# numz/ComfyUI-SeedVR2_VideoUpscaler

Hardware: AMD Instinct MI355X
Metric: upscaled frames/sec (720p->4K, SeedVR2-3B) (higher is better)
Workload: dtype bf16; 1 GPU; cfg3: SeedVR2-3B 32-frame 720p->4K clip (padded to 33 = 4n+1 for encode + DiT, 32 decoded), VAE tiled 1024/128; vae_tiled=True, parallelism=dp1, weights=random-init SeedVR2-3B + video_vae_v3 architecture (seeded)

## Files before the change

comfyui-seedvr2_videoupscaler_amd/csrc/svr_conv_halo2.hip:

```cpp
#include "svr_common.h"
#include "../../include/seedvr2_hip.h"
#include <type_traits>

namespace svr {

constexpr int CG_TX = 32, CG_HX = CG_TX + 2;
constexpr int CG_BUNIT = 128 * 64;
constexpr int CG_NB = 8;
constexpr int CG_D = 4;
static_assert(CG_D < CG_NB, "ring slot of unit k + D must not hold a unit still being read");

template <int TY, int MODE> struct cg_geom {
    static constexpr int MTW = MODE == 3 ? 8 : 4;
    static constexpr int NT = MODE == 3 ? 256 : TY * 32;
    static constexpr int HY = TY + 2;
    static constexpr int ROWS = CG_HX * HY;
    static constexpr int ACHUNKS = ROWS * 4;
    static constexpr int PIECES = (ACHUNKS + NT - 1) / NT;
    static constexpr int ABUF = MODE == 3 ? PIECES * NT * 16 : ROWS * 64;
    static constexpr int BOFF = 2 * ABUF;
    static constexpr int EP_ROWS = MODE ? 4 : 8;
    static constexpr int EP_BYTES = EP_ROWS * 32 * 528;
    static constexpr int THIN_PITCH = 272;
    static constexpr int MAIN = MODE == 2 ? TY * 32 * THIN_PITCH : (MODE == 1 || MODE == 3 ? BOFF : BOFF + CG_NB * CG_BUNIT);
    static constexpr int LDS = MAIN > EP_BYTES ? MAIN : EP_BYTES;
    static_assert(MODE == 3 || PIECES <= 7, "the next halo must have landed before interval 8");
};

template <int N> SVR_DEVICE void cg_wait_vmcnt() { asm volatile("s_waitcnt vmcnt(%0)" ::"n"(N) : "memory"); }
template <int OFF> SVR_DEVICE void cg_rd2(bf16x8 (&r)[2], unsigned a0) {
    const unsigned a1 = a0 ^ 32u;
    asm volatile("ds_read_b128 %0, %2 offset:%4\n\tds_read_b128 %1, %3 offset:%4"
                 : "=&v"(r[0]), "=&v"(r[1]) : "v"(a0), "v"(a1), "n"(OFF) : "memory");
}
template <int N> SVR_DEVICE void cg_wait_rows(bf16x8 (&a)[2]) {
    asm volatile("s_waitcnt lgkmcnt(%2)" : "+v"(a[0]), "+v"(a[1]) : "n"(N));
    __builtin_amdgcn_sched_barrier(0);
}
template <int N> SVR_DEVICE void cg_wait_rows(bf16x8 (&a)[2], bf16x8 (&b)[2]) {
    asm volatile("s_waitcnt lgkmcnt(%4)" : "+v"(a[0]), "+v"(a[1]), "+v"(b[0]), "+v"(b[1]) : "n"(N));
    __builtin_amdgcn_sched_barrier(0);
}
template <int N> SVR_DEVICE void cg_wait_rows(bf16x8 (&a)[2], bf16x8 (&b)[2], bf16x8 (&c)[2], bf16x8 (&d)[2], bf16x8 (&e)[2],
                                              bf16x8 (&f)[2], bf16x8 (&g)[2], bf16x8 (&h)[2]) {
    asm volatile("s_waitcnt lgkmcnt(%16)"
                 : "+v"(a[0]), "+v"(a[1]), "+v"(b[0]), "+v"(b[1]), "+v"(c[0]), "+v"(c[1]), "+v"(d[0]), "+v"(d[1]),
                   "+v"(e[0]), "+v"(e[1]), "+v"(f[0]), "+v"(f[1]), "+v"(g[0]), "+v"(g[1]), "+v"(h[0]), "+v"(h[1]) : "n"(N));
    __builtin_amdgcn_sched_barrier(0);
}
template <int N> SVR_DEVICE void cg_wait_w(bf16x8 (&w)[2][2]) {
    asm volatile("s_waitcnt vmcnt(%4)" : "+v"(w[0][0]), "+v"(w[0][1]), "+v"(w[1][0]), "+v"(w[1][1]) : "n"(N));
    __builtin_amdgcn_sched_barrier(0);
}

#ifdef SVR_ABLATIONS
__device__ unsigned long long g_conv_tl[4096][4];
__device__ unsigned long long g_conv_ep[4096][16];
#endif
template <int TY, int MODE, int DBG = 0>
__global__ __launch_bounds__((cg_geom<TY, MODE>::NT), (MODE == 3 ? 1 : 2)) void conv_halo2_kernel(const svr_gemm_args a, const int band_rows) {
#ifndef SVR_ABLATIONS
    static_assert(DBG == 0, "measurement variants (results invalid on purpose) exist only in -DSVR_ABLATIONS builds; the product library instantiates DBG = 0");
#endif
    typedef cg_geom<TY, MODE> G;
    constexpr bool WREG = MODE == 1 || MODE == 3, W8 = MODE == 3, THIN = MODE == 2;
    constexpr int CG_TY = TY, CG_ROWS = G::ROWS, CG_ABUF = G::ABUF, CG_ACHUNKS = G::ACHUNKS, CG_PIECES = G::PIECES,
                  CG_BOFF = G::BOFF, NT = G::NT;
    constexpr int MTW = G::MTW, NTW = 2;
    extern __shared__ __attribute__((aligned(16))) char smem[];
    typedef __attribute__((ext_vector_type(16))) float f32x16_t;

    const svr_conv_geom& g = a.conv;
    const int tid = threadIdx.x;
#ifdef SVR_ABLATIONS
    if constexpr ((DBG & 256) != 0) { if (tid == 0 && blockIdx.x < 4096) g_conv_tl[blockIdx.x][0] = __builtin_amdgcn_s_memtime(); }
#endif
    const int lane = tid & 63;
    const int wave = __builtin_amdgcn_readfirstlane(tid >> 6);
    const int grp = wave >> 2;
    const int wm = wave >> 1, wn = wave & 1;

    const int tiles_x = (g.W + CG_TX - 1) / CG_TX;
    const int tiles_y = (g.H + CG_TY - 1) / CG_TY;
    const int tiles_n = a.N / 128;
    int tl;
    {
        const int nwg = gridDim.x, bid = blockIdx.x;
        const int xcd = bid & 7, j = bid >> 3, q = nwg >> 3, r = nwg & 7;
        tl = (xcd < r ? xcd * (q + 1) : r * (q + 1) + (xcd - r) * q) + j;
    }
    const int tn = tl % tiles_n;
    int rr = tl / tiles_n;
    const int tx = rr % tiles_x; rr /= tiles_x;
    int ty, to;
    if (band_rows > 0 && band_rows < tiles_y) {
        const int per_band = band_rows * g.To;
        const int b = rr / per_band;
        const int rows_b = min(band_rows, tiles_y - b * band_rows);
        const int r2 = rr - b * per_band;
        to = r2 / rows_b;
        ty = b * band_rows + (r2 - to * rows_b);
    } else {
        ty = rr % tiles_y;
        to = rr / tiles_y;
    }
    const int y0 = ty * CG_TY, x0 = tx * CG_TX, n0 = tn * 128;

    const int cpk = THIN ? 1 : g.Cin / 32;
    const int nA = g.kt * cpk;
    const int P = nA * 9;
    const int64_t frame_bytes = (int64_t)g.H * g.W * g.Cin * 2;
    const int srow = tid >> 2, spos = tid & 3;
    const char* wbase = (const char*)a.W + (int64_t)(n0 + srow) * a.K * 2 + ((spos ^ ((srow >> 2) & 3)) * 16);
    uint32_t poff[CG_PIECES];
    uint32_t akeys = 0;
#pragma unroll
    for (int q = 0; q < CG_PIECES; ++q) {
        const int row = q * (NT / 4) + srow;
        const int hy = row / CG_HX, hx = row - hy * CG_HX;
        const int y = y0 - 1 + hy, x = x0 - 1 + hx;
        const bool ok = row < CG_ROWS && (unsigned)y < (unsigned)g.H && (unsigned)x < (unsigned)g.W;
        poff[q] = ok ? (uint32_t)(y * g.W + x) : 0xffffffffu;
        akeys |= (uint32_t)(spos ^ ((hx >> 2) & 3)) << (2 * q);
    }
    char* const wave_dst = smem + wave * 1024;

    auto frame_ptr = [&](int s) -> const char* {
        const int dt = s / cpk;
        const int c0 = (s - dt * cpk) * 32;
        int f = to + dt - g.pt;
        const char* basep = (const char*)a.A;
        if (f < 0) {
            if (g.halo != nullptr) { basep = (const char*)g.halo; f += g.halo_frames; }
            else f = 0;
        }
        return basep + (int64_t)f * frame_bytes + c0 * 2;
    };
    auto stage_a_piece = [&](auto qc, const char* fptr, int buf) {
        constexpr int Q = decltype(qc)::value;
        if (Q * NT + wave * 64 >= CG_ACHUNKS) return false;
        const int ck = (akeys >> (2 * Q)) & 3;
        const char* src = poff[Q] == 0xffffffffu ? (const char*)g.zeros
                                                 : fptr + ((int64_t)poff[Q] * g.Cin + ck * 8) * 2;
        if constexpr (!(DBG & 2))
            if (Q * NT + tid < CG_ACHUNKS) glds16(src, wave_dst + buf * CG_ABUF + Q * (NT * 16));
        return true;
    };
    auto stage_b = [&](int s, int tap, int slot) {
        const int dt = s / cpk;
        const int c0 = (s - dt * cpk) * 32;
        const int64_t koff = ((int64_t)(dt * 9 + tap) * g.Cin + c0) * 2;
        glds16(wbase + koff, wave_dst + CG_BOFF + slot * CG_BUNIT);
    };

    const int l31 = lane & 31, hi = lane >> 5;
    int rd_a0[3], rd_b0;
#pragma unroll
    for (int dx = 0; dx < 3; ++dx)
        rd_a0[dx] = (wm * MTW * CG_HX + l31) * 64 + ((hi ^ (((dx + l31) >> 2) & 3)) << 4);
    rd_b0 = CG_BOFF + (wn * 64 + l31) * 64 + ((hi ^ ((l31 >> 2) & 3)) << 4);

    f32x16_t acc[MTW][NTW];
#pragma unroll
    for (int y = 0; y < MTW; ++y)
#pragma unroll
        for (int z = 0; z < NTW; ++z)
#pragma unroll
            for (int e = 0; e < 16; ++e) acc[y][z][e] = 0.f;
    bf16x8 ar0[2], ar1[2], ar2[2], ar3[2], ar4[2], ar5[2], wf[NTW][2];
    bf16x8 ar6[2], ar7[2], ar8[2], ar9[2];

    auto reads = [&](auto jc, int s, int k) {
        constexpr int J = decltype(jc)::value;
        constexpr int DY = J % 3, DX = J / 3;
        int ra = rd_a0[DX] + (s & 1) * CG_ABUF;
        int rb = rd_b0 + (k & (CG_NB - 1)) * CG_BUNIT;
        asm volatile("" : "+v"(ra), "+v"(rb));
#pragma unroll
        for (int ks = 0; ks < 2; ++ks) {
            const char* pa = smem + (ra ^ (ks << 5));
            const char* pb = smem + (rb ^ (ks << 5));
            if constexpr (DY == 0) {
                ar0[ks] = *(const bf16x8*)(pa + (0 * CG_HX + DX) * 64);
                ar1[ks] = *(const bf16x8*)(pa + (1 * CG_HX + DX) * 64);
                ar2[ks] = *(const bf16x8*)(pa + (2 * CG_HX + DX) * 64);
                ar3[ks] = *(const bf16x8*)(pa + (3 * CG_HX + DX) * 64);
            } else if constexpr (DY == 1) {
                ar4[ks] = *(const bf16x8*)(pa + (4 * CG_HX + DX) * 64);
            } else {
                ar5[ks] = *(const bf16x8*)(pa + (5 * CG_HX + DX) * 64);
            }
#pragma unroll
            for (int nt = 0; nt < NTW; ++nt) wf[nt][ks] = *(const bf16x8*)(pb + nt * (32 * 64));
        }
    };
    auto mfma_core = [&](const bf16x8 (&r0)[2], const bf16x8 (&r1)[2], const bf16x8 (&r2)[2], const bf16x8 (&r3)[2]) {
#define SVR_MM(KS, R, MT, NT) \
        acc[MT][NT] = __builtin_amdgcn_mfma_f32_32x32x16_bf16(wf[NT][KS], R[KS], acc[MT][NT], 0, 0, 0)
        __builtin_amdgcn_s_setprio(1);
        SVR_MM(0, r0, 0, 0); SVR_MM(0, r0, 0, 1); SVR_MM(0, r1, 1, 0); SVR_MM(0, r1, 1, 1);
        SVR_MM(0, r2, 2, 0); SVR_MM(0, r2, 2, 1); SVR_MM(0, r3, 3, 0); SVR_MM(0, r3, 3, 1);
        SVR_MM(1, r0, 0, 0); SVR_MM(1, r0, 0, 1); SVR_MM(1, r1, 1, 0); SVR_MM(1, r1, 1, 1);
        SVR_MM(1, r2, 2, 0); SVR_MM(1, r2, 2, 1); SVR_MM(1, r3, 3, 0); SVR_MM(1, r3, 3, 1);
        __builtin_amdgcn_s_setprio(0);
#undef SVR_MM
    };
    auto mfmas = [&](auto jc) {
        constexpr int DY = decltype(jc)::value % 3;
        if constexpr (DY == 0) mfma_core(ar0, ar1, ar2, ar3);
        else if constexpr (DY == 1) mfma_core(ar1, ar2, ar3, ar4);
        else mfma_core(ar2, ar3, ar4, ar5);
    };

    if constexpr (THIN) {
        constexpr int TP = G::THIN_PITCH;
        static_assert(NT == 256, "one voxel per thread");
        const int taps = g.kt * 9;
        {
            const int y = y0 + (tid >> 5), x = x0 + (tid & 31);
            char* rowp = smem + tid * TP;
            const int64_t fpix = (int64_t)g.H * g.W;
            uint2 vv[32];
#pragma unroll
            for (int tap = 0; tap < 32; ++tap) {
                uint2 v = make_uint2(0u, 0u);
                if (tap < taps) {
                    const int dt = tap / 9, r = tap - dt * 9, dy = r / 3, dx = r - dy * 3;
                    const int ys = y + dy - 1, xs = x + dx - 1;
                    if ((unsigned)ys < (unsigned)g.H && (unsigned)xs < (unsigned)g.W) {
                        int f = to + dt - g.pt;
                        const char* basep = (const char*)a.A;
                        if (f < 0) {
                            if (g.halo != nullptr) { basep = (const char*)g.halo; f += g.halo_frames; }
                            else f = 0;
                        }
                        v = *(const uint2*)(basep + ((int64_t)f * fpix + (int64_t)ys * g.W + xs) * 8);
                    }
                }
                vv[tap] = v;
            }
#pragma unroll
            for (int tap = 0; tap < 32; tap += 2)
                *(uint4*)(rowp + tap * 8) = make_uint4(vv[tap].x, vv[tap].y, vv[tap + 1].x, vv[tap + 1].y);
        }
        __syncthreads();
        const int nks = (taps * 4 + 15) >> 4;
        const char* wrow0 = (const char*)a.W + ((int64_t)(n0 + wn * 64 + l31) * a.K + hi * 8) * 2;
        const char* arow0 = smem + ((wm * MTW) * 32 + l31) * TP + hi * 16;
#pragma unroll
        for (int ks = 0; ks < 8; ++ks) {
            if (ks < nks) {
                const bf16x8 b0 = *(const bf16x8*)(wrow0 + ks * 32);
                const bf16x8 b1 = *(const bf16x8*)(wrow0 + (int64_t)32 * a.K * 2 + ks * 32);
#pragma unroll
                for (int mt = 0; mt < MTW; ++mt) {
                    const bf16x8 av = *(const bf16x8*)(arow0 + mt * 32 * TP + ks * 32);
                    acc[mt][0] = __builtin_amdgcn_mfma_f32_32x32x16_bf16(b0, av, acc[mt][0], 0, 0, 0);
                    acc[mt][1] = __builtin_amdgcn_mfma_f32_32x32x16_bf16(b1, av, acc[mt][1], 0, 0, 0);
                }
            }
        }
        __syncthreads();
    } else
    if constexpr (WREG) {
        const int64_t nstride = (int64_t)P * 2048;
        const char* wp0 = (const char*)a.W_frag + (int64_t)(n0 / 32 + wn * 2) * nstride;
        const char* wp1 = wp0 + nstride;
        const int voff = lane * 16;
        bf16x8 w0[NTW][2], w1[NTW][2], w2[NTW][2];
        auto wload = [&](bf16x8 (&w)[NTW][2], int k) {
            if constexpr ((DBG & 32) != 0) k &= 3;
            auto uniform_ptr = [](const char* p) {
                const uint64_t u = (uint64_t)p;
                const uint32_t lo = __builtin_amdgcn_readfirstlane((uint32_t)u), hi = __builtin_amdgcn_readfirstlane((uint32_t)(u >> 32));
                return (const char*)(((uint64_t)hi << 32) | lo);
            };
            const char* p0 = uniform_ptr(wp0 + (int64_t)min(k, P - 1) * 2048);
            const char* p1 = uniform_ptr(wp1 + (int64_t)min(k, P - 1) * 2048);
            if constexpr ((DBG & 1) != 0 && W8) {
                if (k > 2) return;
            } else if constexpr (DBG & 1) {
                const bf16x8 z = {0, 0, 0, 0, 0, 0, 0, 0};
                w[0][0] = z; w[0][1] = z; w[1][0] = z; w[1][1] = z;
                return;
            }
            asm volatile("global_load_dwordx4 %0, %1, %2" : "=v"(w[0][0]) : "v"(voff), "s"(p0) : "memory");
            asm volatile("global_load_dwordx4 %0, %1, %2 offset:1024" : "=v"(w[0][1]) : "v"(voff), "s"(p0) : "memory");
            asm volatile("global_load_dwordx4 %0, %1, %2" : "=v"(w[1][0]) : "v"(voff), "s"(p1) : "memory");
            asm volatile("global_load_dwordx4 %0, %1, %2 offset:1024" : "=v"(w[1][1]) : "v"(voff), "s"(p1) : "memory");
        };
        auto reads_a = [&](auto jc, int s) {
            constexpr int J = decltype(jc)::value;
            constexpr int DY = J % 3, DX = J / 3;
            if constexpr ((DBG & 64) != 0) { if (s > 0) return; }
            int ra = rd_a0[DX] + (s & 1) * CG_ABUF;
            asm volatile("" : "+v"(ra));
#pragma unroll
            for (int ks = 0; ks < 2; ++ks) {
                const char* pa = smem + (ra ^ (ks << 5));
                if constexpr (DY == 0) {
                    ar0[ks] = *(const bf16x8*)(pa + (0 * CG_HX + DX) * 64);
                    ar1[ks] = *(const bf16x8*)(pa + (1 * CG_HX + DX) * 64);
                    ar2[ks] = *(const bf16x8*)(pa + (2 * CG_HX + DX) * 64);
                    ar3[ks] = *(const bf16x8*)(pa + (3 * CG_HX + DX) * 64);
                } else if constexpr (DY == 1) {
                    ar4[ks] = *(const bf16x8*)(pa + (4 * CG_HX + DX) * 64);
                } else {
                    ar5[ks] = *(const bf16x8*)(pa + (5 * CG_HX + DX) * 64);
                }
            }
        };
        auto mfma_w = [&](const bf16x8 (&w)[NTW][2], const bf16x8 (&r0)[2], const bf16x8 (&r1)[2],
                          const bf16x8 (&r2)[2], const bf16x8 (&r3)[2]) {
#define SVR_MM(KS, R, MT, NT) \
            acc[MT][NT] = __builtin_amdgcn_mfma_f32_32x32x16_bf16(w[NT][KS], R[KS], acc[MT][NT], 0, 0, 0)
            SVR_MM(0, r0, 0, 0); SVR_MM(0, r0, 0, 1); SVR_MM(0, r1, 1, 0); SVR_MM(0, r1, 1, 1);
            SVR_MM(0, r2, 2, 0); SVR_MM(0, r2, 2, 1); SVR_MM(0, r3, 3, 0); SVR_MM(0, r3, 3, 1);
            SVR_MM(1, r0, 0, 0); SVR_MM(1, r0, 0, 1); SVR_MM(1, r1, 1, 0); SVR_MM(1, r1, 1, 1);
            SVR_MM(1, r2, 2, 0); SVR_MM(1, r2, 2, 1); SVR_MM(1, r3, 3, 0); SVR_MM(1, r3, 3, 1);
#undef SVR_MM
        };
        if constexpr (W8) {
        const unsigned lds0 = (unsigned)(uintptr_t)(__attribute__((address_space(3))) char*)smem;
        unsigned fa[3];
#pragma unroll
        for (int dx = 0; dx < 3; ++dx) fa[dx] = lds0 + (unsigned)rd_a0[dx];
        auto stage_full = [&](auto qc, const char* fptr, int buf) {
            constexpr int Q = decltype(qc)::value;
            const int ck = (akeys >> (2 * Q)) & 3;
            const char* src = (poff[Q] == 0xffffffffu || fptr == nullptr) ? (const char*)g.zeros
                                                                          : fptr + ((int64_t)poff[Q] * g.Cin + ck * 8) * 2;
            glds16(src, wave_dst + buf * CG_ABUF + Q * (NT * 16));
        };
        static_assert(CG_PIECES == 10, "piece schedule below is written for ten pieces, two per interval 0..4");
        constexpr bool ABL_NO_DMA = (DBG & 16) != 0, ABL_NO_W = (DBG & 1) != 0, ABL_NO_RD = (DBG & 64) != 0;
#define SVR_RD(ROW, R, DXV, BUFOFF) do { if constexpr (!ABL_NO_RD) cg_rd2<((R) * CG_HX + (DXV)) * 64>(ROW, fa[DXV] + (BUFOFF)); } while (0)
#define SVR_MM(W, KS, ROW, MT, NTI) \
        acc[MT][NTI] = __builtin_amdgcn_mfma_f32_32x32x16_bf16(W[NTI][KS], ROW[KS], acc[MT][NTI], 0, 0, 0)
#define SVR_MM8(W, RA, MA, RB, MB) \
        SVR_MM(W, 0, RA, MA, 0); SVR_MM(W, 0, RA, MA, 1); SVR_MM(W, 0, RB, MB, 0); SVR_MM(W, 0, RB, MB, 1); \
        SVR_MM(W, 1, RA, MA, 0); SVR_MM(W, 1, RA, MA, 1); SVR_MM(W, 1, RB, MB, 0); SVR_MM(W, 1, RB, MB, 1)
        auto interval8 = [&](auto jc, int s, const char* fnext, bf16x8 (&wc)[NTW][2], bf16x8 (&wn_)[NTW][2]) {
            constexpr int J = decltype(jc)::value;
            constexpr int DY = J % 3, DX = J / 3;
            const int k = s * 9 + J;
            const unsigned cur = (unsigned)((s & 1) * CG_ABUF), nxt = (unsigned)(((s + 1) & 1) * CG_ABUF);
            constexpr int NPC[9] = {2, 2, 2, 2, 2, 0, 0, 0, 0};
            constexpr int NV = 4 + NPC[(J + 8) % 9] + NPC[(J + 7) % 9];
            if constexpr (DY == 0) {
                cg_wait_rows<0>(ar0, ar1, ar2, ar3, ar4, ar5, ar6, ar7);
                SVR_RD(ar8, 8, DX, cur);
                SVR_RD(ar9, 9, DX, cur);
            } else if constexpr (DY == 1 && J != 7) {
                cg_wait_rows<4>(ar8);
            } else if constexpr (DY == 2 && J != 8) {
                cg_wait_rows<4>(ar9);
            }
            if constexpr (!ABL_NO_DMA && !ABL_NO_W) cg_wait_w<NV>(wc);
            else if constexpr (ABL_NO_DMA && !ABL_NO_W) cg_wait_w<4>(wc);
            if constexpr (J == 7) SVR_RD(ar0, 0, 0, nxt);
            __builtin_amdgcn_sched_barrier(0);
            if constexpr (DY == 0) { SVR_MM8(wc, ar0, 0, ar1, 1); }
            else if constexpr (DY == 1) { SVR_MM8(wc, ar1, 0, ar2, 1); }
            else { SVR_MM8(wc, ar2, 0, ar3, 1); }
            __builtin_amdgcn_sched_barrier(0);
            if constexpr (DX < 2) {
                if constexpr (DY == 0) SVR_RD(ar0, 0, DX + 1, cur);
                else if constexpr (DY == 1) SVR_RD(ar1, 1, DX + 1, cur);
                else { SVR_RD(ar2, 2, DX + 1, cur); SVR_RD(ar3, 3, DX + 1, cur); }
            } else {
                if constexpr (DY == 1) SVR_RD(ar1, 1, 0, nxt);
                else if constexpr (DY == 2) { SVR_RD(ar2, 2, 0, nxt); SVR_RD(ar3, 3, 0, nxt); }
            }
            wload(wn_, k + 2);
            __builtin_amdgcn_sched_barrier(0);
            if constexpr (DY == 0) { SVR_MM8(wc, ar2, 2, ar3, 3); }
            else if constexpr (DY == 1) { SVR_MM8(wc, ar3, 2, ar4, 3); }
            else { SVR_MM8(wc, ar4, 2, ar5, 3); }
            __builtin_amdgcn_sched_barrier(0);
            if constexpr (DY == 2) {
                if constexpr (DX < 2) { SVR_RD(ar4, 4, DX + 1, cur); SVR_RD(ar5, 5, DX + 1, cur); }
                else { SVR_RD(ar4, 4, 0, nxt); SVR_RD(ar5, 5, 0, nxt); }
            }
            if constexpr (J < 5 && !ABL_NO_DMA) {
                stage_full(std::integral_constant<int, (J < 5 ? 2 * J : 0)>{}, fnext, (s + 1) & 1);
                stage_full(std::integral_constant<int, (J < 5 ? 2 * J + 1 : 0)>{}, fnext, (s + 1) & 1);
            }
            __builtin_amdgcn_sched_barrier(0);
            if constexpr (DY == 0) { SVR_MM8(wc, ar4, 4, ar5, 5); }
            else if constexpr (DY == 1) { SVR_MM8(wc, ar5, 4, ar6, 5); }
            else { SVR_MM8(wc, ar6, 4, ar7, 5); }
            __builtin_amdgcn_sched_barrier(0);
            if constexpr (DY == 2) {
                if constexpr (DX < 2) { SVR_RD(ar6, 6, DX + 1, cur); SVR_RD(ar7, 7, DX + 1, cur); }
                else { SVR_RD(ar6, 6, 0, nxt); SVR_RD(ar7, 7, 0, nxt); }
            }
            __builtin_amdgcn_sched_barrier(0);
            if constexpr (DY == 0) { SVR_MM8(wc, ar6, 6, ar7, 7); }
            else if constexpr (DY == 1) { SVR_MM8(wc, ar7, 6, ar8, 7); }
            else { SVR_MM8(wc, ar8, 6, ar9, 7); }
            __builtin_amdgcn_sched_barrier(0);
            if constexpr (J == 6) {
                cg_wait_rows<0>(ar8, ar9);
                if constexpr (!ABL_NO_DMA && !ABL_NO_W) cg_wait_vmcnt<8>();
                __builtin_amdgcn_s_barrier();
                __builtin_amdgcn_sched_barrier(0);
            }
        };
        {
            const char* f0 = frame_ptr(0);
            stage_full(std::integral_constant<int, 0>{}, f0, 0);
            stage_full(std::integral_constant<int, 1>{}, f0, 0);
            stage_full(std::integral_constant<int, 2>{}, f0, 0);
            stage_full(std::integral_constant<int, 3>{}, f0, 0);
            stage_full(std::integral_constant<int, 4>{}, f0, 0);
            stage_full(std::integral_constant<int, 5>{}, f0, 0);
            stage_full(std::integral_constant<int, 6>{}, f0, 0);
            stage_full(std::integral_constant<int, 7>{}, f0, 0);
            stage_full(std::integral_constant<int, 8>{}, f0, 0);
            stage_full(std::integral_constant<int, 9>{}, f0, 0);
            wload(w0, 0);
            wload(w1, 1);
            if constexpr (ABL_NO_W) wload(w2, 2);
            __builtin_amdgcn_sched_barrier(0);
#pragma unroll
            for (int y = 0; y < MTW; ++y)
#pragma unroll
                for (int z = 0; z < NTW; ++z) asm volatile("" : "+a"(acc[y][z]));
            cg_wait_vmcnt<0>();
            __builtin_amdgcn_s_barrier();
            __builtin_amdgcn_sched_barrier(0);
#define SVR_RD0(ROW, R) cg_rd2<((R) * CG_HX) * 64>(ROW, fa[0])
            SVR_RD0(ar0, 0); SVR_RD0(ar1, 1); SVR_RD0(ar2, 2); SVR_RD0(ar3, 3);
            SVR_RD0(ar4, 4); SVR_RD0(ar5, 5); SVR_RD0(ar6, 6); SVR_RD0(ar7, 7);
            if constexpr (ABL_NO_RD) { SVR_RD0(ar8, 8); SVR_RD0(ar9, 9); }
#undef SVR_RD0
        }
#ifdef SVR_ABLATIONS
        if constexpr ((DBG & 256) != 0) { if (tid == 0 && blockIdx.x < 4096) g_conv_tl[blockIdx.x][1] = __builtin_amdgcn_s_memtime(); }
#endif
        for (int s = 0; s < nA; ++s) {
            const char* fnext = s + 1 < nA ? frame_ptr((DBG & 128) ? 0 : s + 1) : nullptr;
            interval8(std::integral_constant<int, 0>{}, s, fnext, w0, w2);
            interval8(std::integral_constant<int, 1>{}, s, fnext, w1, w0);
            interval8(std::integral_constant<int, 2>{}, s, fnext, w2, w1);
            interval8(std::integral_constant<int, 3>{}, s, fnext, w0, w2);
            interval8(std::integral_constant<int, 4>{}, s, fnext, w1, w0);
            interval8(std::integral_constant<int, 5>{}, s, fnext, w2, w1);
            interval8(std::integral_constant<int, 6>{}, s, fnext, w0, w2);
            interval8(std::integral_constant<int, 7>{}, s, fnext, w1, w0);
            interval8(std::integral_constant<int, 8>{}, s, fnext, w2, w1);
        }
        cg_wait_vmcnt<0>();
        asm volatile("s_waitcnt lgkmcnt(0)" ::: "memory");
        __builtin_amdgcn_sched_barrier(0);
#undef SVR_RD
#undef SVR_MM
#undef SVR_MM8
        } else {
        bool a_prev3 = false;
        auto interval3 = [&](auto jc, int s, const char* fnext, const bf16x8 (&wc)[NTW][2], bf16x8 (&wn_)[NTW][2]) {
            constexpr int J = decltype(jc)::value;
            constexpr int DY = J % 3;
            const int k = s * 9 + J;
            bool a_issued = false;
            if constexpr (J < CG_PIECES && !(DBG & 16)) {
                if (s + 1 < nA) a_issued = stage_a_piece(std::integral_constant<int, (J < CG_PIECES ? J : 0)>{}, fnext, (s + 1) & 1);
            }
            wload(wn_, k + 2);
            reads_a(jc, s);
            {
                const int n = 8 + (a_issued ? 1 : 0) + (a_prev3 ? 1 : 0);
                if (n == 10) cg_wait_vmcnt<10>(); else if (n == 9) cg_wait_vmcnt<9>(); else cg_wait_vmcnt<8>();
            }
            a_prev3 = a_issued;
            asm volatile("s_waitcnt lgkmcnt(0)" ::: "memory");
            __builtin_amdgcn_sched_barrier(0);
            if (grp == 0) __builtin_amdgcn_s_setprio(2); else __builtin_amdgcn_s_setprio(1);
            if constexpr (DY == 0) mfma_w(wc, ar0, ar1, ar2, ar3);
            else if constexpr (DY == 1) mfma_w(wc, ar1, ar2, ar3, ar4);
            else mfma_w(wc, ar2, ar3, ar4, ar5);
            __builtin_amdgcn_s_setprio(0);
            __builtin_amdgcn_sched_barrier(0);
            if constexpr (J == 8) {
                if (s + 1 < nA) cg_wait_vmcnt<8>(); else cg_wait_vmcnt<0>();
                if constexpr (!(DBG & 8)) __builtin_amdgcn_s_barrier();
                __builtin_amdgcn_sched_barrier(0);
            }
        };
        {
            const char* f0 = frame_ptr(0);
            stage_a_piece(std::integral_constant<int, 0>{}, f0, 0);
            stage_a_piece(std::integral_constant<int, 1>{}, f0, 0);
            stage_a_piece(std::integral_constant<int, 2>{}, f0, 0);
            stage_a_piece(std::integral_constant<int, 3>{}, f0, 0);
            stage_a_piece(std::integral_constant<int, 4>{}, f0, 0);
            if constexpr (CG_PIECES > 5) stage_a_piece(std::integral_constant<int, (CG_PIECES > 5 ? 5 : 0)>{}, f0, 0);
            static_assert(CG_PIECES <= 6, "prologue stages at most six pieces");
            if constexpr ((DBG & 16) != 0) {
                stage_a_piece(std::integral_constant<int, 0>{}, f0, 1);
                stage_a_piece(std::integral_constant<int, 1>{}, f0, 1);
                stage_a_piece(std::integral_constant<int, 2>{}, f0, 1);
                stage_a_piece(std::integral_constant<int, 3>{}, f0, 1);
                stage_a_piece(std::integral_constant<int, 4>{}, f0, 1);
                if constexpr (CG_PIECES > 5) stage_a_piece(std::integral_constant<int, (CG_PIECES > 5 ? 5 : 0)>{}, f0, 1);
            }
            wload(w0, 0);
            wload(w1, 1);
            cg_wait_vmcnt<0>();
            __builtin_amdgcn_s_barrier();
            __builtin_amdgcn_sched_barrier(0);
        }
#ifdef SVR_ABLATIONS
        if constexpr ((DBG & 256) != 0) { if (tid == 0 && blockIdx.x < 4096) g_conv_tl[blockIdx.x][1] = __builtin_amdgcn_s_memtime(); }
#endif
        for (int s = 0; s < nA; ++s) {
            const char* fnext = frame_ptr((DBG & 128) ? 0 : min(s + 1, nA - 1));
            interval3(std::integral_constant<int, 0>{}, s, fnext, w0, w2);
            interval3(std::integral_constant<int, 1>{}, s, fnext, w1, w0);
            interval3(std::integral_constant<int, 2>{}, s, fnext, w2, w1);
            interval3(std::integral_constant<int, 3>{}, s, fnext, w0, w2);
            interval3(std::integral_constant<int, 4>{}, s, fnext, w1, w0);
            interval3(std::integral_constant<int, 5>{}, s, fnext, w2, w1);
            interval3(std::integral_constant<int, 6>{}, s, fnext, w0, w2);
            interval3(std::integral_constant<int, 7>{}, s, fnext, w1, w0);
            interval3(std::integral_constant<int, 8>{}, s, fnext, w2, w1);
        }
        }
    } else {
    {
        const char* f0 = frame_ptr(0);
        stage_a_piece(std::integral_constant<int, 0>{}, f0, 0);
        stage_a_piece(std::integral_constant<int, 1>{}, f0, 0);
        stage_a_piece(std::integral_constant<int, 2>{}, f0, 0);
        stage_a_piece(std::integral_constant<int, 3>{}, f0, 0);
        stage_a_piece(std::integral_constant<int, 4>{}, f0, 0);
#pragma unroll
        for (int u = 0; u < CG_D; ++u) stage_b(0, (u % 3) * 3 + u / 3, u);
        cg_wait_vmcnt<0>();
        __builtin_amdgcn_s_barrier();
    }
    if (grp == 0) {
        reads(std::integral_constant<int, 0>{}, 0, 0);
        asm volatile("s_waitcnt lgkmcnt(0)" ::: "memory");
    }
    __builtin_amdgcn_sched_barrier(0);

    bool a_prev = false;
    auto interval = [&](auto jc, int s, const char* fnext) {
        constexpr int J = decltype(jc)::value;
        const int k = s * 9 + J;
        if (grp == 0) {
            mfmas(jc);
            if constexpr (J + 1 < 9) reads(std::integral_constant<int, (J + 1) % 9>{}, s, k + 1);
            else if (s + 1 < nA) reads(std::integral_constant<int, 0>{}, s + 1, k + 1);
        } else {
            reads(jc, s, k);
        }
        bool a_issued = false;
        if constexpr (J < CG_PIECES) {
            if (s + 1 < nA) a_issued = stage_a_piece(std::integral_constant<int, (J < CG_PIECES ? J : 0)>{}, fnext, (s + 1) & 1);
        }
        const bool b_issued = k + CG_D < P;
        if (b_issued) {
            constexpr int JU = (J + CG_D) % 9;
            stage_b(s + (J + CG_D) / 9, (JU % 3) * 3 + JU / 3, (k + CG_D) & (CG_NB - 1));
        }
        static_assert(CG_D == 4, "counts below are written for a prefetch distance of 4");
        if (b_issued) {
            const int n = 2 + (a_issued ? 1 : 0) + (a_prev ? 1 : 0);
            if (n == 4) cg_wait_vmcnt<4>(); else if (n == 3) cg_wait_vmcnt<3>(); else cg_wait_vmcnt<2>();
        } else {
            cg_wait_vmcnt<0>();
        }
        a_prev = a_issued;
        asm volatile("s_waitcnt lgkmcnt(0)" ::: "memory");
        __builtin_amdgcn_sched_barrier(0);
        if (grp == 1) mfmas(jc);
        __builtin_amdgcn_sched_barrier(0);
        __builtin_amdgcn_s_barrier();
        __builtin_amdgcn_sched_barrier(0);
    };

    for (int s = 0; s < nA; ++s) {
        const char* fnext = frame_ptr(min(s + 1, nA - 1));
        interval(std::integral_constant<int, 0>{}, s, fnext);
        interval(std::integral_constant<int, 1>{}, s, fnext);
        interval(std::integral_constant<int, 2>{}, s, fnext);
        interval(std::integral_constant<int, 3>{}, s, fnext);
        interval(std::integral_constant<int, 4>{}, s, fnext);
        interval(std::integral_constant<int, 5>{}, s, fnext);
        interval(std::integral_constant<int, 6>{}, s, fnext);
        interval(std::integral_constant<int, 7>{}, s, fnext);
        interval(std::integral_constant<int, 8>{}, s, fnext);
    }

    }

#ifdef SVR_ABLATIONS
    if constexpr ((DBG & 256) != 0) { if (tid == 0 && blockIdx.x < 4096) g_conv_tl[blockIdx.x][2] = __builtin_amdgcn_s_memtime(); }
#endif
    constexpr int EP_PITCH = 528;
    const int hi4 = hi * 4;
    f32x4 bias_lo = {0.f, 0.f, 0.f, 0.f}, bias_hi = {0.f, 0.f, 0.f, 0.f};
    if (a.bias) {
        bias_lo = *(const f32x4*)(a.bias + n0 + (tid & 15) * 8);
        bias_hi = *(const f32x4*)(a.bias + n0 + (tid & 15) * 8 + 4);
    }
#ifdef SVR_ABLATIONS
#define SVR_EP_STAMP(i) if constexpr ((DBG & 256) != 0) { if (tid == 0 && blockIdx.x < 4096) g_conv_ep[blockIdx.x][i] = __builtin_amdgcn_s_memtime(); }
#else
#define SVR_EP_STAMP(i)
#endif
    SVR_EP_STAMP(0)
    const bool resid_gate = a.epilogue == SVR_EPI_RESID_GATE;
    double gs0 = 0.0, gq0 = 0.0, gs1 = 0.0, gq1 = 0.0;
    constexpr int EP_ROWS = G::EP_ROWS;
    constexpr int NPASS = MTW / 2;
    static_assert(TY / EP_ROWS == NPASS && EP_ROWS * 32 * 16 == 8 * NT, "MTW / 2 passes, eight store iterations each");
    auto ep_body = [&](auto fc) {
        constexpr int F = decltype(fc)::value;
        constexpr bool RT = F < 0, F_RESID = !RT && (F & 1), F_GN = !RT && (F & 2);
        const bool with_resid = RT ? (resid_gate && a.resid != nullptr) : F_RESID;
        const int ko = RT ? a.out_f32 : ((F & 4) != 0 ? SVR_STORE_H16 : SVR_STORE_BF16);
        const int kr = RT ? a.resid_f32 : ((F & 8) != 0 ? SVR_STORE_H16 : SVR_STORE_BF16);
        const bool o32 = ko == SVR_STORE_FP32, r32 = kr == SVR_STORE_FP32;
        const bool with_gn = RT ? a.gn_partial != nullptr : F_GN;
        constexpr bool PRE = W8 && !RT && F_RESID;
        uint4 rpre[2][8];
        auto resid_prefetch = [&](auto pc, uint4 (&dst)[8]) {
            constexpr int P = decltype(pc)::value;
            const int n_ = n0 + (tid & 15) * 8;
#pragma unroll
            for (int q = 0; q < 8; ++q) {
                const int vox = (q * NT + tid) >> 4;
                const int r = vox >> 5;
                const int y = y0 + (r >> 1) * MTW + 2 * P + (r & 1), x = x0 + (vox & 31);
                const int64_t m_ = ((int64_t)to * g.H + min(y, g.H - 1)) * g.W + min(x, g.W - 1);
                dst[q] = *(const uint4*)((const bf16_t*)a.resid + m_ * a.ldr + n_);
            }
        };
        if constexpr (PRE) resid_prefetch(std::integral_constant<int, 0>{}, rpre[0]);
#pragma unroll
        for (int pass = 0; pass < NPASS; ++pass) {
#pragma unroll
            for (int j = 0; j < 2; ++j) {
                char* row = smem + ((wm * 2 + j) * 32 + l31) * EP_PITCH;
#pragma unroll
                for (int nt = 0; nt < NTW; ++nt) {
                    const f32x16_t v = acc[2 * pass + j][nt];
#pragma unroll
                    for (int gq = 0; gq < 4; ++gq) {
                        const f32x4 o = {v[4 * gq], v[4 * gq + 1], v[4 * gq + 2], v[4 * gq + 3]};
                        *(f32x4*)(row + (wn * 64 + nt * 32 + 8 * gq + hi4) * 4) = o;
                    }
                }
            }
            SVR_EP_STAMP(1 + 3 * pass)
            if constexpr ((DBG & 512) != 0) __syncthreads(); else lds_barrier();
            SVR_EP_STAMP(2 + 3 * pass)
            if constexpr (PRE) {
                if (pass + 1 < NPASS) {
                    if (pass == 0) resid_prefetch(std::integral_constant<int, 1>{}, rpre[1]);
                    else if (pass == 1) resid_prefetch(std::integral_constant<int, 2>{}, rpre[0]);
                    else if (pass == 2) resid_prefetch(std::integral_constant<int, 3>{}, rpre[1]);
                }
            }
            const int n = n0 + (tid & 15) * 8;
#pragma unroll
            for (int half = 0; half < 2; ++half) {
            f32x4 lo[4], hi_[4];
            uint4 rr8[4];
            f32x4 rf0[4], rf1[4];
            int64_t mrow[4];
            bool ok[4];
#pragma unroll
            for (int it = 0; it < 4; ++it) {
                const int vox = ((half * 4 + it) * NT + tid) >> 4;
                const int r = vox >> 5;
                const int y = y0 + (r >> 1) * MTW + 2 * pass + (r & 1), x = x0 + (vox & 31);
                ok[it] = y < g.H && x < g.W;
                if constexpr ((DBG & 4) != 0) ok[it] = false;
                mrow[it] = ((int64_t)to * g.H + min(y, g.H - 1)) * g.W + min(x, g.W - 1);
                lo[it] = *(const f32x4*)(smem + vox * EP_PITCH + (tid & 15) * 32);
                hi_[it] = *(const f32x4*)(smem + vox * EP_PITCH + (tid & 15) * 32 + 16);
            }
            if (with_resid) {
                if constexpr (RT) {
                    if (!r32) {
#pragma unroll
                        for (int it = 0; it < 4; ++it) rr8[it] = *(const uint4*)((const bf16_t*)a.resid + mrow[it] * a.ldr + n);
                    }
                } else if (r32) {
#pragma unroll
                    for (int it = 0; it < 4; ++it) {
                        const float* rp = (const float*)a.resid + mrow[it] * a.ldr + n;
                        rf0[it] = *(const f32x4*)rp;
                        rf1[it] = *(const f32x4*)(rp + 4);
                    }
                } else {
                    if constexpr (PRE) {
#pragma unroll
                        for (int it = 0; it < 4; ++it) rr8[it] = rpre[pass & 1][half * 4 + it];
                    } else {
#pragma unroll
                        for (int it = 0; it < 4; ++it) rr8[it] = *(const uint4*)((const bf16_t*)a.resid + mrow[it] * a.ldr + n);
                    }
                }
            }
#pragma unroll
            for (int it = 0; it < 4; ++it) {
                float f[8] = {lo[it][0] + bias_lo[0], lo[it][1] + bias_lo[1], lo[it][2] + bias_lo[2], lo[it][3] + bias_lo[3],
                              hi_[it][0] + bias_hi[0], hi_[it][1] + bias_hi[1], hi_[it][2] + bias_hi[2], hi_[it][3] + bias_hi[3]};
                if constexpr (RT) {
                    if (a.epilogue == SVR_EPI_BIAS_SILU) {
#pragma unroll
                        for (int e = 0; e < 8; ++e) f[e] = silu(f[e]);
                    }
                    if (resid_gate && a.gate) {
#pragma unroll
                        for (int e = 0; e < 8; ++e) f[e] *= a.gate[n + e];
                    }
                }
                if (with_resid) {
                    float r8[8];
                    if (r32) {
                        if constexpr (RT) {
                            const float* rp = (const float*)a.resid + mrow[it] * a.ldr + n;
                            rf0[0] = *(const f32x4*)rp;
                            rf1[0] = *(const f32x4*)(rp + 4);
                        }
#pragma unroll
                        for (int e = 0; e < 4; ++e) { r8[e] = rf0[RT ? 0 : it][e]; r8[4 + e] = rf1[RT ? 0 : it][e]; }
                    } else if (kr == SVR_STORE_H16) {
                        unpack8h(rr8[it], r8);
                    } else {
                        unpack8(rr8[it], r8);
                    }
#pragma unroll
                    for (int e = 0; e < 8; ++e) f[e] += r8[e];
                }
                if (o32) {
                    if (ok[it]) {
                        float* cp = (float*)a.C + mrow[it] * a.ldc + n;
                        *(float4*)cp = make_float4(f[0], f[1], f[2], f[3]);
                        *(float4*)(cp + 4) = make_float4(f[4], f[5], f[6], f[7]);
                        if (with_gn) {
                            gn_accumulate4(gs0, gq0, f[0], f[1], f[2], f[3]);
                            gn_accumulate4(gs1, gq1, f[4], f[5], f[6], f[7]);
                        }
                    }
                } else {
                    const uint4 pk = ko == SVR_STORE_H16 ? pack8h(f) : pack8(f);
                    if (ok[it]) *(uint4*)((bf16_t*)a.C + mrow[it] * a.ldc + n) = pk;
                    if (with_gn && ok[it]) {
                        float r[8];
                        if (ko == SVR_STORE_H16) unpack8h(pk, r); else unpack8(pk, r);
                        gn_accumulate4(gs0, gq0, r[0], r[1], r[2], r[3]);
                        gn_accumulate4(gs1, gq1, r[4], r[5], r[6], r[7]);
                    }
                }
            }
            }
            SVR_EP_STAMP(3 + 3 * pass)
            if (pass + 1 < NPASS) { if constexpr ((DBG & 512) != 0) __syncthreads(); else lds_barrier(); }
        }
    };
    const bool wr = resid_gate && a.resid != nullptr;
    if (a.epilogue != SVR_EPI_BIAS_SILU && a.gate == nullptr && a.out_f32 != SVR_STORE_FP32 && !(wr && a.resid_f32 == SVR_STORE_FP32) &&
        (DBG == 0 || (!a.out_f32 && !a.resid_f32))) {
        const int F = (wr ? 1 : 0) | (a.gn_partial != nullptr ? 2 : 0) | (a.out_f32 == SVR_STORE_H16 ? 4 : 0) |
                      (wr && a.resid_f32 == SVR_STORE_H16 ? 8 : 0);
        switch (F) {
#define SVR_EP_CASE(v) case v: ep_body(std::integral_constant<int, v>{}); break;
            SVR_EP_CASE(0) SVR_EP_CASE(1) SVR_EP_CASE(2) SVR_EP_CASE(3)
            default:
                if constexpr (DBG == 0) switch (F) {
                    SVR_EP_CASE(4) SVR_EP_CASE(5) SVR_EP_CASE(6) SVR_EP_CASE(7) SVR_EP_CASE(9) SVR_EP_CASE(11) SVR_EP_CASE(13) SVR_EP_CASE(15)
                    default: break;
                }
                break;
#undef SVR_EP_CASE
        }
    } else {
        ep_body(std::integral_constant<int, -1>{});
    }
    if (a.gn_partial) {
        __syncthreads();
        static_assert(NT * 32 + 32 * 16 <= G::LDS, "statistics staging fits the kernel's LDS");
        double4* red = (double4*)smem;
        double2* qsum = (double2*)(smem + NT * 32);
        red[tid] = make_double4(gs0, gq0, gs1, gq1);
        __syncthreads();
        if (tid < 32) {
            const int c = tid >> 1, h = tid & 1;
            double s = 0.0, q = 0.0;
            for (int j = 0; j < NT / 16; ++j) {
                const double4 v = red[(j << 4) | c];
                s += h ? v.z : v.x;
                q += h ? v.w : v.y;
            }
            qsum[tid] = make_double2(s, q);
        }
        __syncthreads();
        const int qpg = (a.N / a.gn_groups) >> 2;
        if (tid < 32 / qpg) {
            double s = 0.0, q = 0.0;
            for (int i = 0; i < qpg; ++i) { s += qsum[tid * qpg + i].x; q += qsum[tid * qpg + i].y; }
// ... 94 lines not shown
```

Measured before the change: 3.587 frames/s.

## Switch halo conv kernel from 32x32x16 to 16x16x32 bf16 MFMA tiles

Replaces each 32x32x16 MFMA with four 16x16x32 MFMAs over a 2x2 sub-tile accumulator layout. LDS read addressing, weight-fragment load offsets, the thin-K path and the epilogue scatter are rewritten to match the new lane mapping (16-lane rows, 4 column groups, k-halves 1024 bytes apart instead of XOR-swizzled). The aim is to use the higher-throughput or lower-latency 16x16 MFMA shape and to simplify the addressing. It adds an s_nop pad after the main loop and relies on the pre-packed weight fragment layout matching the new offsets, which is a correctness risk.

```diff
diff --git a/comfyui-seedvr2_videoupscaler_amd/csrc/svr_conv_halo2.hip b/comfyui-seedvr2_videoupscaler_amd/csrc/svr_conv_halo2.hip
--- a/comfyui-seedvr2_videoupscaler_amd/csrc/svr_conv_halo2.hip
+++ b/comfyui-seedvr2_videoupscaler_amd/csrc/svr_conv_halo2.hip
@@ -29,9 +29,20 @@
 
 template <int N> SVR_DEVICE void cg_wait_vmcnt() { asm volatile("s_waitcnt vmcnt(%0)" ::"n"(N) : "memory"); }
 template <int OFF> SVR_DEVICE void cg_rd2(bf16x8 (&r)[2], unsigned a0) {
-    const unsigned a1 = a0 ^ 32u;
-    asm volatile("ds_read_b128 %0, %2 offset:%4\n\tds_read_b128 %1, %3 offset:%4"
-                 : "=&v"(r[0]), "=&v"(r[1]) : "v"(a0), "v"(a1), "n"(OFF) : "memory");
+    asm volatile("ds_read_b128 %0, %2 offset:%3\n\tds_read_b128 %1, %2 offset:%4"
+                 : "=&v"(r[0]), "=&v"(r[1]) : "v"(a0), "n"(OFF), "n"(OFF + 1024) : "memory");
+}
+SVR_DEVICE void cg_mm4(f32x4 (&c)[2][2], const bf16x8 (&w)[2], const bf16x8 (&r)[2]) {
+    c[0][0] = __builtin_amdgcn_mfma_f32_16x16x32_bf16(w[0], r[0], c[0][0], 0, 0, 0);
+    c[0][1] = __builtin_amdgcn_mfma_f32_16x16x32_bf16(w[1], r[0], c[0][1], 0, 0, 0);
+    c[1][0] = __builtin_amdgcn_mfma_f32_16x16x32_bf16(w[0], r[1], c[1][0], 0, 0, 0);
+    c[1][1] = __builtin_amdgcn_mfma_f32_16x16x32_bf16(w[1], r[1], c[1][1], 0, 0, 0);
+}
+SVR_DEVICE void cg_mm4_inplace(f32x4 (&c)[2][2], const bf16x8 (&w)[2], const bf16x8 (&r)[2]) {
+    asm volatile("v_mfma_f32_16x16x32_bf16 %0, %1, %2, %0" : "+v"(c[0][0]) : "v"(w[0]), "v"(r[0]));
+    asm volatile("v_mfma_f32_16x16x32_bf16 %0, %1, %2, %0" : "+v"(c[0][1]) : "v"(w[1]), "v"(r[0]));
+    asm volatile("v_mfma_f32_16x16x32_bf16 %0, %1, %2, %0" : "+v"(c[1][0]) : "v"(w[0]), "v"(r[1]));
+    asm volatile("v_mfma_f32_16x16x32_bf16 %0, %1, %2, %0" : "+v"(c[1][1]) : "v"(w[1]), "v"(r[1]));
 }
 template <int N> SVR_DEVICE void cg_wait_rows(bf16x8 (&a)[2]) {
     asm volatile("s_waitcnt lgkmcnt(%2)" : "+v"(a[0]), "+v"(a[1]) : "n"(N));
@@ -68,7 +79,6 @@
                   CG_BOFF = G::BOFF, NT = G::NT;
     constexpr int MTW = G::MTW, NTW = 2;
     extern __shared__ __attribute__((aligned(16))) char smem[];
-    typedef __attribute__((ext_vector_type(16))) float f32x16_t;
 
     const svr_conv_geom& g = a.conv;
     const int tid = threadIdx.x;
@@ -153,20 +163,20 @@
         glds16(wbase + koff, wave_dst + CG_BOFF + slot * CG_BUNIT);
     };
 
-    const int l31 = lane & 31, hi = lane >> 5;
+    const int l15 = lane & 15, c4 = lane >> 4;
     int rd_a0[3], rd_b0;
 #pragma unroll
     for (int dx = 0; dx < 3; ++dx)
-        rd_a0[dx] = (wm * MTW * CG_HX + l31) * 64 + ((hi ^ (((dx + l31) >> 2) & 3)) << 4);
-    rd_b0 = CG_BOFF + (wn * 64 + l31) * 64 + ((hi ^ ((l31 >> 2) & 3)) << 4);
-
-    f32x16_t acc[MTW][NTW];
+        rd_a0[dx] = (wm * MTW * CG_HX + l15) * 64 + ((c4 ^ (((dx + l15) >> 2) & 3)) << 4);
+    rd_b0 = CG_BOFF + (wn * 64 + l15) * 64 + ((c4 ^ ((l15 >> 2) & 3)) << 4);
+
+    f32x4 acc[MTW][NTW][2][2];
 #pragma unroll
     for (int y = 0; y < MTW; ++y)
 #pragma unroll
         for (int z = 0; z < NTW; ++z)
 #pragma unroll
-            for (int e = 0; e < 16; ++e) acc[y][z][e] = 0.f;
+            for (int e = 0; e < 16; ++e) acc[y][z][e >> 3][(e >> 2) & 1][e & 3] = 0.f;
     bf16x8 ar0[2], ar1[2], ar2[2], ar3[2], ar4[2], ar5[2], wf[NTW][2];
     bf16x8 ar6[2], ar7[2], ar8[2], ar9[2];
 
@@ -178,8 +188,8 @@
         asm volatile("" : "+v"(ra), "+v"(rb));
 #pragma unroll
         for (int ks = 0; ks < 2; ++ks) {
-            const char* pa = smem + (ra ^ (ks << 5));
-            const char* pb = smem + (rb ^ (ks << 5));
+            const char* pa = smem + ra + ks * 1024;
+            const char* pb = smem + rb + ks * 1024;
             if constexpr (DY == 0) {
                 ar0[ks] = *(const bf16x8*)(pa + (0 * CG_HX + DX) * 64);
                 ar1[ks] = *(const bf16x8*)(pa + (1 * CG_HX + DX) * 64);
@@ -195,15 +205,10 @@
         }
     };
     auto mfma_core = [&](const bf16x8 (&r0)[2], const bf16x8 (&r1)[2], const bf16x8 (&r2)[2], const bf16x8 (&r3)[2]) {
-#define SVR_MM(KS, R, MT, NT) \
-        acc[MT][NT] = __builtin_amdgcn_mfma_f32_32x32x16_bf16(wf[NT][KS], R[KS], acc[MT][NT], 0, 0, 0)
         __builtin_amdgcn_s_setprio(1);
-        SVR_MM(0, r0, 0, 0); SVR_MM(0, r0, 0, 1); SVR_MM(0, r1, 1, 0); SVR_MM(0, r1, 1, 1);
-        SVR_MM(0, r2, 2, 0); SVR_MM(0, r2, 2, 1); SVR_MM(0, r3, 3, 0); SVR_MM(0, r3, 3, 1);
-        SVR_MM(1, r0, 0, 0); SVR_MM(1, r0, 0, 1); SVR_MM(1, r1, 1, 0); SVR_MM(1, r1, 1, 1);
-        SVR_MM(1, r2, 2, 0); SVR_MM(1, r2, 2, 1); SVR_MM(1, r3, 3, 0); SVR_MM(1, r3, 3, 1);
+        cg_mm4(acc[0][0], wf[0], r0); cg_mm4(acc[0][1], wf[1], r0); cg_mm4(acc[1][0], wf[0], r1); cg_mm4(acc[1][1], wf[1], r1);
+        cg_mm4(acc[2][0], wf[0], r2); cg_mm4(acc[2][1], wf[1], r2); cg_mm4(acc[3][0], wf[0], r3); cg_mm4(acc[3][1], wf[1], r3);
         __builtin_amdgcn_s_setprio(0);
-#undef SVR_MM
     };
     auto mfmas = [&](auto jc) {
         constexpr int DY = decltype(jc)::value % 3;
@@ -244,19 +249,22 @@
                 *(uint4*)(rowp + tap * 8) = make_uint4(vv[tap].x, vv[tap].y, vv[tap + 1].x, vv[tap + 1].y);
         }
         __syncthreads();
-        const int nks = (taps * 4 + 15) >> 4;
-        const char* wrow0 = (const char*)a.W + ((int64_t)(n0 + wn * 64 + l31) * a.K + hi * 8) * 2;
-        const char* arow0 = smem + ((wm * MTW) * 32 + l31) * TP + hi * 16;
-#pragma unroll
-        for (int ks = 0; ks < 8; ++ks) {
+        const int nks = (taps * 4 + 31) >> 5;
+        const char* wrow0 = (const char*)a.W + ((int64_t)(n0 + wn * 64 + l15) * a.K + c4 * 8) * 2;
+        const char* arow0 = smem + ((wm * MTW) * 32 + l15) * TP + c4 * 16;
+#pragma unroll
+        for (int ks = 0; ks < 4; ++ks) {
             if (ks < nks) {
-                const bf16x8 b0 = *(const bf16x8*)(wrow0 + ks * 32);
-                const bf16x8 b1 = *(const bf16x8*)(wrow0 + (int64_t)32 * a.K * 2 + ks * 32);
+                bf16x8 b[NTW][2];
+#pragma unroll
+                for (int q = 0; q < 2 * NTW; ++q) b[q >> 1][q & 1] = *(const bf16x8*)(wrow0 + (int64_t)(16 * q) * a.K * 2 + ks * 64);
 #pragma unroll
                 for (int mt = 0; mt < MTW; ++mt) {
-                    const bf16x8 av = *(const bf16x8*)(arow0 + mt * 32 * TP + ks * 32);
-                    acc[mt][0] = __builtin_amdgcn_mfma_f32_32x32x16_bf16(b0, av, acc[mt][0], 0, 0, 0);
-                    acc[mt][1] = __builtin_amdgcn_mfma_f32_32x32x16_bf16(b1, av, acc[mt][1], 0, 0, 0);
+                    bf16x8 av[2];
+                    av[0] = *(const bf16x8*)(arow0 + mt * 32 * TP + ks * 64);
+                    av[1] = *(const bf16x8*)(arow0 + (mt * 32 + 16) * TP + ks * 64);
+                    cg_mm4(acc[mt][0], b[0], av);
+                    cg_mm4(acc[mt][1], b[1], av);
                 }
             }
         }
@@ -266,7 +274,7 @@
         const int64_t nstride = (int64_t)P * 2048;
         const char* wp0 = (const char*)a.W_frag + (int64_t)(n0 / 32 + wn * 2) * nstride;
         const char* wp1 = wp0 + nstride;
-        const int voff = lane * 16;
+        const int voff = c4 * 512 + l15 * 16;
         bf16x8 w0[NTW][2], w1[NTW][2], w2[NTW][2];
         auto wload = [&](bf16x8 (&w)[NTW][2], int k) {
             if constexpr ((DBG & 32) != 0) k &= 3;
@@ -285,9 +293,9 @@
                 return;
             }
             asm volatile("global_load_dwordx4 %0, %1, %2" : "=v"(w[0][0]) : "v"(voff), "s"(p0) : "memory");
-            asm volatile("global_load_dwordx4 %0, %1, %2 offset:1024" : "=v"(w[0][1]) : "v"(voff), "s"(p0) : "memory");
+            asm volatile("global_load_dwordx4 %0, %1, %2 offset:256" : "=v"(w[0][1]) : "v"(voff), "s"(p0) : "memory");
             asm volatile("global_load_dwordx4 %0, %1, %2" : "=v"(w[1][0]) : "v"(voff), "s"(p1) : "memory");
-            asm volatile("global_load_dwordx4 %0, %1, %2 offset:1024" : "=v"(w[1][1]) : "v"(voff), "s"(p1) : "memory");
+            asm volatile("global_load_dwordx4 %0, %1, %2 offset:256" : "=v"(w[1][1]) : "v"(voff), "s"(p1) : "memory");
         };
         auto reads_a = [&](auto jc, int s) {
             constexpr int J = decltype(jc)::value;
@@ -297,7 +305,7 @@
             asm volatile("" : "+v"(ra));
 #pragma unroll
             for (int ks = 0; ks < 2; ++ks) {
-                const char* pa = smem + (ra ^ (ks << 5));
+                const char* pa = smem + ra + ks * 1024;
                 if constexpr (DY == 0) {
                     ar0[ks] = *(const bf16x8*)(pa + (0 * CG_HX + DX) * 64);
                     ar1[ks] = *(const bf16x8*)(pa + (1 * CG_HX + DX) * 64);
@@ -312,13 +320,10 @@
         };
         auto mfma_w = [&](const bf16x8 (&w)[NTW][2], const bf16x8 (&r0)[2], const bf16x8 (&r1)[2],
                           const bf16x8 (&r2)[2], const bf16x8 (&r3)[2]) {
-#define SVR_MM(KS, R, MT, NT) \
-            acc[MT][NT] = __builtin_amdgcn_mfma_f32_32x32x16_bf16(w[NT][KS], R[KS], acc[MT][NT], 0, 0, 0)
-            SVR_MM(0, r0, 0, 0); SVR_MM(0, r0, 0, 1); SVR_MM(0, r1, 1, 0); SVR_MM(0, r1, 1, 1);
-            SVR_MM(0, r2, 2, 0); SVR_MM(0, r2, 2, 1); SVR_MM(0, r3, 3, 0); SVR_MM(0, r3, 3, 1);
-            SVR_MM(1, r0, 0, 0); SVR_MM(1, r0, 0, 1); SVR_MM(1, r1, 1, 0); SVR_MM(1, r1, 1, 1);
-            SVR_MM(1, r2, 2, 0); SVR_MM(1, r2, 2, 1); SVR_MM(1, r3, 3, 0); SVR_MM(1, r3, 3, 1);
-#undef SVR_MM
+            cg_mm4_inplace(acc[0][0], w[0], r0); cg_mm4_inplace(acc[0][1], w[1], r0);
+            cg_mm4_inplace(acc[1][0], w[0], r1); cg_mm4_inplace(acc[1][1], w[1], r1);
+            cg_mm4_inplace(acc[2][0], w[0], r2); cg_mm4_inplace(acc[2][1], w[1], r2);
+            cg_mm4_inplace(acc[3][0], w[0], r3); cg_mm4_inplace(acc[3][1], w[1], r3);
         };
         if constexpr (W8) {
         const unsigned lds0 = (unsigned)(uintptr_t)(__attribute__((address_space(3))) char*)smem;
@@ -335,11 +340,8 @@
         static_assert(CG_PIECES == 10, "piece schedule below is written for ten pieces, two per interval 0..4");
         constexpr bool ABL_NO_DMA = (DBG & 16) != 0, ABL_NO_W = (DBG & 1) != 0, ABL_NO_RD = (DBG & 64) != 0;
 #define SVR_RD(ROW, R, DXV, BUFOFF) do { if constexpr (!ABL_NO_RD) cg_rd2<((R) * CG_HX + (DXV)) * 64>(ROW, fa[DXV] + (BUFOFF)); } while (0)
-#define SVR_MM(W, KS, ROW, MT, NTI) \
-        acc[MT][NTI] = __builtin_amdgcn_mfma_f32_32x32x16_bf16(W[NTI][KS], ROW[KS], acc[MT][NTI], 0, 0, 0)
 #define SVR_MM8(W, RA, MA, RB, MB) \
-        SVR_MM(W, 0, RA, MA, 0); SVR_MM(W, 0, RA, MA, 1); SVR_MM(W, 0, RB, MB, 0); SVR_MM(W, 0, RB, MB, 1); \
-        SVR_MM(W, 1, RA, MA, 0); SVR_MM(W, 1, RA, MA, 1); SVR_MM(W, 1, RB, MB, 0); SVR_MM(W, 1, RB, MB, 1)
+        cg_mm4(acc[MA][0], W[0], RA); cg_mm4(acc[MA][1], W[1], RA); cg_mm4(acc[MB][0], W[0], RB); cg_mm4(acc[MB][1], W[1], RB)
         auto interval8 = [&](auto jc, int s, const char* fnext, bf16x8 (&wc)[NTW][2], bf16x8 (&wn_)[NTW][2]) {
             constexpr int J = decltype(jc)::value;
             constexpr int DY = J % 3, DX = J / 3;
@@ -426,7 +428,8 @@
 #pragma unroll
             for (int y = 0; y < MTW; ++y)
 #pragma unroll
-                for (int z = 0; z < NTW; ++z) asm volatile("" : "+a"(acc[y][z]));
+                for (int z = 0; z < NTW; ++z)
+                    asm volatile("" : "+a"(acc[y][z][0][0]), "+a"(acc[y][z][0][1]), "+a"(acc[y][z][1][0]), "+a"(acc[y][z][1][1]));
             cg_wait_vmcnt<0>();
             __builtin_amdgcn_s_barrier();
             __builtin_amdgcn_sched_barrier(0);
@@ -455,7 +458,6 @@
         asm volatile("s_waitcnt lgkmcnt(0)" ::: "memory");
         __builtin_amdgcn_sched_barrier(0);
 #undef SVR_RD
-#undef SVR_MM
 #undef SVR_MM8
         } else {
         bool a_prev3 = false;
@@ -526,6 +528,7 @@
             interval3(std::integral_constant<int, 7>{}, s, fnext, w1, w0);
             interval3(std::integral_constant<int, 8>{}, s, fnext, w2, w1);
         }
+        asm volatile("s_nop 7\n\ts_nop 7" ::: "memory");
         }
     } else {
     {
@@ -601,7 +604,6 @@
     if constexpr ((DBG & 256) != 0) { if (tid == 0 && blockIdx.x < 4096) g_conv_tl[blockIdx.x][2] = __builtin_amdgcn_s_memtime(); }
 #endif
     constexpr int EP_PITCH = 528;
-    const int hi4 = hi * 4;
     f32x4 bias_lo = {0.f, 0.f, 0.f, 0.f}, bias_hi = {0.f, 0.f, 0.f, 0.f};
     if (a.bias) {
         bias_lo = *(const f32x4*)(a.bias + n0 + (tid & 15) * 8);
@@ -645,15 +647,14 @@
         for (int pass = 0; pass < NPASS; ++pass) {
 #pragma unroll
             for (int j = 0; j < 2; ++j) {
-                char* row = smem + ((wm * 2 + j) * 32 + l31) * EP_PITCH;
-#pragma unroll
-                for (int nt = 0; nt < NTW; ++nt) {
-                    const f32x16_t v = acc[2 * pass + j][nt];
-#pragma unroll
-                    for (int gq = 0; gq < 4; ++gq) {
-                        const f32x4 o = {v[4 * gq], v[4 * gq + 1], v[4 * gq + 2], v[4 * gq + 3]};
-                        *(f32x4*)(row + (wn * 64 + nt * 32 + 8 * gq + hi4) * 4) = o;
-                    }
+#pragma unroll
+                for (int vh = 0; vh < 2; ++vh) {
+                    char* row = smem + ((wm * 2 + j) * 32 + vh * 16 + l15) * EP_PITCH;
+#pragma unroll
+                    for (int nt = 0; nt < NTW; ++nt)
+#pragma unroll
+                        for (int ch = 0; ch < 2; ++ch)
+                            *(f32x4*)(row + (wn * 64 + nt * 32 + ch * 16 + c4 * 4) * 4) = acc[2 * pass + j][nt][vh][ch];
                 }
             }
             SVR_EP_STAMP(1 + 3 * pass)
```

Result: faster. 3.764 frames/s, median of 6 (+4.9%).
